# fpthink/PDGN

Hardware: AMD Instinct MI355X
Metric: generator+D step points/sec (B=35, 256->2048 pts) (higher is better)
Workload: dtype f32; 1 GPU; PDGNet_v2 G+D iteration (models/PDGNet_v2.py:171-256), chair-shaped synthetic batch, per-GPU batch 35, 256->2048 pts, random-init weights; global_batch=35, parallelism=dp1, losses_finite=True, hipgraph=False, issue=list

## Files before the change

### pdgn_amd/csrc/bnact.hip

```cpp
#include "common.h"

#include "bn_geom.h"
#define ACT_NONE 0
#define ACT_RELU 1
#define ACT_LEAKY 2

__device__ __forceinline__ float act_fwd(float z, int act) {
    if (act == ACT_RELU) return fmaxf(z, 0.f);
    if (act == ACT_LEAKY) return z > 0.f ? z : 0.01f * z;
    return z;
}
__device__ __forceinline__ float act_grad(float z, int act) {
    if (act == ACT_RELU) return z > 0.f ? 1.f : 0.f;
    if (act == ACT_LEAKY) return z > 0.f ? 1.f : 0.01f;
    return 1.f;
}

struct ClGeom {
    int cg, cgb, rl;
};

__global__ __launch_bounds__(BN_THREADS) void cl_stats_kernel(long long R, int C, int cgb, int rows_per_block,
                                                              const float *__restrict__ x,
                                                              float *__restrict__ part) {
// ... 635 lines not shown
    float acc[12];
#pragma unroll
    for (int i = 0; i < 12; ++i) acc[i] = 0.f;
    if (ok)
        for (long long m = m0 + rlane; m < m1; m += rl) {
            const size_t ox = (size_t)m * k * C + c, ou = (size_t)m * k * C + 2 * c;
            float2 xv[KM];
            float4 uv[KM / 2], wv[KM / 2], gv[KM / 2];
#pragma unroll
            for (int s = 0; s < KM; ++s)
                if (KT || s < k) xv[s] = *reinterpret_cast<const float2 *>(x + ox + (size_t)s * C);
#pragma unroll
            for (int p = 0; p < KM / 2; ++p)
                if (KT || p < P) {
                    uv[p] = *reinterpret_cast<const float4 *>(u + ou + (size_t)p * Cu);
                    if (w) wv[p] = *reinterpret_cast<const float4 *>(w + ou + (size_t)p * Cu);
                    gv[p] = *reinterpret_cast<const float4 *>(dy + ou + (size_t)p * Cu);
                }
            if (!w) {
                float h0[KM], h1[KM];
                float mx0 = -INFINITY, mx1 = -INFINITY;
#pragma unroll
                for (int s = 0; s < KM; ++s)
                    if (KT || s < k) {
                        h0[s] = act_fwd(__fmaf_rn(xv[s].x, scx.x, shx.x), act);
                        h1[s] = act_fwd(__fmaf_rn(xv[s].y, scx.y, shx.y), act);
                        mx0 = fmaxf(mx0, h0[s]);
                        mx1 = fmaxf(mx1, h1[s]);
                    }
                float e0 = 0.f, e1 = 0.f;
#pragma unroll
                for (int s = 0; s < KM; ++s)
                    if (KT || s < k) {
                        h0[s] = __expf(h0[s] - mx0);
                        h1[s] = __expf(h1[s] - mx1);
                        e0 += h0[s];
                        e1 += h1[s];
                    }
                const float i0 = 1.0f / e0, i1 = 1.0f / e1;
#pragma unroll
                for (int p = 0; p < KM / 2; ++p)
                    if (KT || p < P) wv[p] = make_float4(h0[p] * i0, h0[P + p] * i0, h1[p] * i1, h1[P + p] * i1);
            }
            float dot0 = 0.f, dot1 = 0.f;
#pragma unroll
            for (int p = 0; p < KM / 2; ++p)
                if (KT || p < P) {
                    const float u4[4] = {uv[p].x, uv[p].y, uv[p].z, uv[p].w}, w4[4] = {wv[p].x, wv[p].y, wv[p].z, wv[p].w};
                    const float g4[4] = {gv[p].x, gv[p].y, gv[p].z, gv[p].w};
                    const float s4[4] = {scu.x, scu.y, scu.z, scu.w}, h4[4] = {shu.x, shu.y, shu.z, shu.w};
                    const float m4[4] = {muu.x, muu.y, muu.z, muu.w}, i4[4] = {isu.x, isu.y, isu.z, isu.w};
                    const float a4[4] = {cau.x, cau.y, cau.z, cau.w}, b4[4] = {cbu.x, cbu.y, cbu.z, cbu.w};
                    float dW[4], o4[4];
#pragma unroll
                    for (int j = 0; j < 4; ++j) {
                        const float z = __fmaf_rn(u4[j], s4[j], h4[j]);
                        dW[j] = g4[j] * act_fwd(z, act);
                        const float dz = g4[j] * w4[j] * act_grad(z, act);
                        if (APPLY) o4[j] = __fmaf_rn(s4[j], dz, -a4[j]) - b4[j] * u4[j];
                        else { acc[4 + j] += dz; acc[8 + j] = __fmaf_rn(dz, (u4[j] - m4[j]) * i4[j], acc[8 + j]); }
                    }
                    if (APPLY) *reinterpret_cast<float4 *>(du + ou + (size_t)p * Cu) = make_float4(o4[0], o4[1], o4[2], o4[3]);
                    dot0 = __fmaf_rn(w4[0], dW[0], __fmaf_rn(w4[1], dW[1], dot0));
                    dot1 = __fmaf_rn(w4[2], dW[2], __fmaf_rn(w4[3], dW[3], dot1));
                    gv[p] = make_float4(dW[0], dW[1], dW[2], dW[3]);
                }
#pragma unroll
            for (int s = 0; s < KM; ++s)
                if (KT || s < k) {
                    const int p = s < P ? s : s - P;
                    const bool hi = s >= P;
                    const float w0 = hi ? wv[p].y : wv[p].x, g0 = hi ? gv[p].y : gv[p].x;
                    const float w1 = hi ? wv[p].w : wv[p].z, g1 = hi ? gv[p].w : gv[p].z;
                    const float da0 = w0 * (g0 - dot0), da1 = w1 * (g1 - dot1);
                    const float dz0 = da0 * act_grad(__fmaf_rn(xv[s].x, scx.x, shx.x), act);
                    const float dz1 = da1 * act_grad(__fmaf_rn(xv[s].y, scx.y, shx.y), act);
                    if (APPLY) {
                        float2 o;
                        o.x = __fmaf_rn(scx.x, dz0, -cax.x) - cbx.x * xv[s].x;
                        o.y = __fmaf_rn(scx.y, dz1, -cax.y) - cbx.y * xv[s].y;
                        *reinterpret_cast<float2 *>(dx + ox + (size_t)s * C) = o;
                    } else {
                        acc[0] += dz0; acc[1] += dz1;
                        acc[2] = __fmaf_rn(dz0, (xv[s].x - mux.x) * isx.x, acc[2]);
                        acc[3] = __fmaf_rn(dz1, (xv[s].y - mux.y) * isx.y, acc[3]);
                    }
                }
        }
    if (APPLY) return;
#pragma unroll
    for (int i = 0; i < 12; ++i) red[i][threadIdx.x] = acc[i];
    __syncthreads();
    if (rlane == 0 && ok) {
        for (int j = 1; j < rl; ++j)
#pragma unroll
            for (int i = 0; i < 12; ++i) acc[i] += red[i][j * cpb + cpl];
        float *px = part_x + (size_t)blockIdx.y * 2 * C, *pu = part_u + (size_t)blockIdx.y * 2 * Cu;
        *reinterpret_cast<float2 *>(px + c) = make_float2(acc[0], acc[1]);
        *reinterpret_cast<float2 *>(px + C + c) = make_float2(acc[2], acc[3]);
        *reinterpret_cast<float4 *>(pu + 2 * c) = make_float4(acc[4], acc[5], acc[6], acc[7]);
        *reinterpret_cast<float4 *>(pu + Cu + 2 * c) = make_float4(acc[8], acc[9], acc[10], acc[11]);
    }
}

static void bw_geometry(long long M, int C, int *cpb, int *gx, int *gy, int *mpb) {
    const int c2 = C / 2;
    int p = 1;
    while (p < c2 && p < BN_THREADS) p <<= 1;
    *cpb = p;
    *gx = (c2 + p - 1) / p;
    const int rl = BN_THREADS / p;
    long long want = 1024 / *gx;
    want = want < 1 ? 1 : want;
    long long rows = (M + want - 1) / want;
    rows = rows < (long long)rl * 4 ? (long long)rl * 4 : rows;
    rows = rows > 4096 ? 4096 : rows;
    rows = (rows + rl - 1) / rl * rl;
    *mpb = (int)rows;
    *gy = (int)((M + rows - 1) / rows);
}

extern "C" long long pdgn_bilateral_scratch_floats(long long m, int k, int c) {
    if (m < 1 || k < 2 || (k & 1) || k > BW_MAXK || c < 2 || (c & 1)) return PDGN_ERR_INVALID;
    int cpb, gx, gy, mpb;
    bw_geometry(m, c, &cpb, &gx, &gy, &mpb);
    return (long long)gy * 6 * c + 6 * c;
}

extern "C" int pdgn_bilateral_weighting_backward(long long m, int k, int c, int act, int training, const float *x,
                                                 const float *stats_x, const float *u, const float *stats_u,
                                                 const float *w, const float *dy, float *scratch, float *bsums_x,
                                                 float *bsums_u, float *dx, float *du, pdgn_stream_t stream) {
    if (m < 1 || k < 2 || (k & 1) || k > BW_MAXK || c < 4 || (c % 4) || act < 0 || act > 2) return PDGN_ERR_INVALID;
    hipStream_t s = (hipStream_t)stream;
    int cpb, gx, gy, mpb;
    bw_geometry(m, c, &cpb, &gx, &gy, &mpb);
    float *part_x = scratch, *part_u = part_x + (size_t)gy * 2 * c;
    float *coef_x = part_u + (size_t)gy * 4 * c, *coef_u = coef_x + 2 * c;
    const dim3 grid(gx, gy), block(BN_THREADS);
#define BW_LAUNCH(KT, AP)                                                                                              \
    hipLaunchKernelGGL((bilateral_bwd_kernel<KT, AP>), grid, block, 0, s, m, k, c, cpb, mpb, act, x, stats_x, u, stats_u, w, \
                       dy, part_x, part_u, coef_x, coef_u, dx, du)
    if (k == 10) BW_LAUNCH(10, false); else if (k == 4) BW_LAUNCH(4, false); else BW_LAUNCH(0, false);
    hipLaunchKernelGGL(cl_bwd_finalize_kernel, dim3(cdiv(c, FIN_CH)), dim3(FIN_CH * FIN_PL), 0, s, m * k, c, gy, training, part_x,
                       stats_x, bsums_x, coef_x);
    hipLaunchKernelGGL(cl_bwd_finalize_kernel, dim3(cdiv(2 * c, FIN_CH)), dim3(FIN_CH * FIN_PL), 0, s, m * (k / 2), 2 * c, gy,
                       training, part_u, stats_u, bsums_u, coef_u);
    if (k == 10) BW_LAUNCH(10, true); else if (k == 4) BW_LAUNCH(4, true); else BW_LAUNCH(0, true);
#undef BW_LAUNCH
    return pdgn_launch_status();
}

#define MP_SPLIT 16

__global__ __launch_bounds__(BN_THREADS) void cl_apply_max_kernel(int N, int C, int cgb, int act,
                                                                  const float *__restrict__ x,
                                                                  const float *__restrict__ stats,
                                                                  float *__restrict__ pmax, int32_t *__restrict__ parg) {
    __shared__ float smax[BN_THREADS][4];
    __shared__ int sarg[BN_THREADS][4];
    const int cgl = threadIdx.x % cgb, rlane = threadIdx.x / cgb, rl = BN_THREADS / cgb;
    const int cgi = blockIdx.x * cgb + cgl;
    const bool cok = cgi * 4 < C;
    const int b = blockIdx.z, sp = blockIdx.y;
    const int per = (N + MP_SPLIT - 1) / MP_SPLIT;
    const int n0 = sp * per, n1 = min(N, n0 + per);
    float best[4] = {-INFINITY, -INFINITY, -INFINITY, -INFINITY};
    int arg[4] = {n0, n0, n0, n0};
    if (cok) {
        float sc[4], sh[4];
        *reinterpret_cast<float4 *>(sc) = *reinterpret_cast<const float4 *>(stats + cgi * 4);
        *reinterpret_cast<float4 *>(sh) = *reinterpret_cast<const float4 *>(stats + C + cgi * 4);
        const float *X = x + ((size_t)b * N) * C + cgi * 4;
        for (int n = n0 + rlane; n < n1; n += rl) {
            float v[4];
            *reinterpret_cast<float4 *>(v) = *reinterpret_cast<const float4 *>(X + (size_t)n * C);
#pragma unroll
            for (int j = 0; j < 4; ++j) {
                const float y = act_fwd(__fmaf_rn(v[j], sc[j], sh[j]), act);
                if (y > best[j]) { best[j] = y; arg[j] = n; }
            }
        }
    }
#pragma unroll
    for (int j = 0; j < 4; ++j) { smax[threadIdx.x][j] = best[j]; sarg[threadIdx.x][j] = arg[j]; }
    __syncthreads();
    if (rlane == 0 && cok) {
        for (int q = 1; q < rl; ++q)
#pragma unroll
            for (int j = 0; j < 4; ++j) {
                const float y = smax[q * cgb + cgl][j];
                const int a = sarg[q * cgb + cgl][j];
                if (y > best[j] || (y == best[j] && a < arg[j])) { best[j] = y; arg[j] = a; }
            }
        const size_t o = ((size_t)b * MP_SPLIT + sp) * C + cgi * 4;
        *reinterpret_cast<float4 *>(pmax + o) = *reinterpret_cast<float4 *>(best);
        *reinterpret_cast<int4 *>(parg + o) = *reinterpret_cast<int4 *>(arg);
    }
}

__global__ void cl_max_finalize_kernel(int B, int C, const float *__restrict__ pmax, const int32_t *__restrict__ parg,
                                       float *__restrict__ ymax, int32_t *__restrict__ yarg) {
    const int e = blockIdx.x * blockDim.x + threadIdx.x;
    if (e >= B * C) return;
    const int b = e / C, c = e % C;
    float best = -INFINITY;
    int arg = 0;
    for (int s = 0; s < MP_SPLIT; ++s) {
        const float y = pmax[((size_t)b * MP_SPLIT + s) * C + c];
        if (y > best) { best = y; arg = parg[((size_t)b * MP_SPLIT + s) * C + c]; }
    }
    ymax[e] = best;
    yarg[e] = arg;
}

__global__ __launch_bounds__(BN_THREADS) void cl_stats_max_kernel(int N, int C, int cgb, const float *__restrict__ x,
                                                                  float *__restrict__ part, float *__restrict__ pmax,
                                                                  int32_t *__restrict__ pargmax, float *__restrict__ pmin,
                                                                  int32_t *__restrict__ pargmin) {
    __shared__ float4 red[4][BN_THREADS];
    __shared__ int4 redi[2][BN_THREADS];
    const int cgl = threadIdx.x % cgb, rlane = threadIdx.x / cgb, rl = BN_THREADS / cgb;
    const int cgi = blockIdx.x * cgb + cgl;
    const bool cok = cgi * 4 < C;
    const int b = blockIdx.z, sp = blockIdx.y;
    const int per = (N + MP_SPLIT - 1) / MP_SPLIT;
    const int n0 = sp * per, n1 = min(N, n0 + per);
    float s[4] = {0.f, 0.f, 0.f, 0.f}, q[4] = {0.f, 0.f, 0.f, 0.f};
    float mx[4] = {-INFINITY, -INFINITY, -INFINITY, -INFINITY}, mn[4] = {INFINITY, INFINITY, INFINITY, INFINITY};
    int amx[4] = {n0, n0, n0, n0}, amn[4] = {n0, n0, n0, n0};
    if (cok) {
        float pv[4];
        *reinterpret_cast<float4 *>(pv) = *reinterpret_cast<const float4 *>(x + cgi * 4);
        const float *X = x + ((size_t)b * N) * C + cgi * 4;
        for (int n = n0 + rlane; n < n1; n += rl) {
            float v[4];
            *reinterpret_cast<float4 *>(v) = *reinterpret_cast<const float4 *>(X + (size_t)n * C);
#pragma unroll
            for (int j = 0; j < 4; ++j) {
                const float d = v[j] - pv[j];
                s[j] += d;
                q[j] = __fmaf_rn(d, d, q[j]);
                if (v[j] > mx[j]) { mx[j] = v[j]; amx[j] = n; }
                if (v[j] < mn[j]) { mn[j] = v[j]; amn[j] = n; }
            }
        }
    }
    red[0][threadIdx.x] = make_float4(s[0], s[1], s[2], s[3]);
    red[1][threadIdx.x] = make_float4(q[0], q[1], q[2], q[3]);
    red[2][threadIdx.x] = make_float4(mx[0], mx[1], mx[2], mx[3]);
    red[3][threadIdx.x] = make_float4(mn[0], mn[1], mn[2], mn[3]);
    redi[0][threadIdx.x] = make_int4(amx[0], amx[1], amx[2], amx[3]);
    redi[1][threadIdx.x] = make_int4(amn[0], amn[1], amn[2], amn[3]);
    __syncthreads();
    if (rlane || !cok) return;
    for (int k = 1; k < rl; ++k) {
        const int t = k * cgb + cgl;
        const float *a = &red[0][t].x, *bq = &red[1][t].x, *c2 = &red[2][t].x, *d2 = &red[3][t].x;
        const int *i2 = &redi[0][t].x, *j2 = &redi[1][t].x;
#pragma unroll
        for (int j = 0; j < 4; ++j) {
            s[j] += a[j];
            q[j] += bq[j];
            if (c2[j] > mx[j] || (c2[j] == mx[j] && i2[j] < amx[j])) { mx[j] = c2[j]; amx[j] = i2[j]; }
            if (d2[j] < mn[j] || (d2[j] == mn[j] && j2[j] < amn[j])) { mn[j] = d2[j]; amn[j] = j2[j]; }
        }
    }
    const size_t blk = (size_t)b * MP_SPLIT + sp;
    float *P = part + blk * 2 * C;
    *reinterpret_cast<float4 *>(P + cgi * 4) = make_float4(s[0], s[1], s[2], s[3]);
    *reinterpret_cast<float4 *>(P + C + cgi * 4) = make_float4(q[0], q[1], q[2], q[3]);
    const size_t o = blk * C + cgi * 4;
    *reinterpret_cast<float4 *>(pmax + o) = make_float4(mx[0], mx[1], mx[2], mx[3]);
    *reinterpret_cast<int4 *>(pargmax + o) = make_int4(amx[0], amx[1], amx[2], amx[3]);
    *reinterpret_cast<float4 *>(pmin + o) = make_float4(mn[0], mn[1], mn[2], mn[3]);
    *reinterpret_cast<int4 *>(pargmin + o) = make_int4(amn[0], amn[1], amn[2], amn[3]);
}

__global__ void cl_max_pick_kernel(int B, int C, int act, const float *__restrict__ stats, const float *__restrict__ pmax,
                                   const int32_t *__restrict__ pargmax, const float *__restrict__ pmin,
                                   const int32_t *__restrict__ pargmin, float *__restrict__ ymax, int32_t *__restrict__ yarg) {
    const int e = blockIdx.x * blockDim.x + threadIdx.x;
    if (e >= B * C) return;
    const int b = e / C, c = e - b * C;
    const float sc = stats[c], sh = stats[C + c];
    const bool up = sc >= 0.f;
    const float *pv = up ? pmax : pmin;
    const int32_t *pa = up ? pargmax : pargmin;
    float best = pv[((size_t)b * MP_SPLIT) * C + c];
    int arg = pa[((size_t)b * MP_SPLIT) * C + c];
    for (int s = 1; s < MP_SPLIT; ++s) {
        const float v = pv[((size_t)b * MP_SPLIT + s) * C + c];
        if (up ? v > best : v < best) { best = v; arg = pa[((size_t)b * MP_SPLIT + s) * C + c]; }
    }
    ymax[e] = act_fwd(__fmaf_rn(best, sc, sh), act);
    yarg[e] = arg;
}

__global__ __launch_bounds__(256) void cl_max_bwd_sums_kernel(int B, int N, int C, int act, int training,
                                                              const float *__restrict__ x, const float *__restrict__ dout,
                                                              const int32_t *__restrict__ yarg, const float *__restrict__ stats,
                                                              float *__restrict__ dz, float *__restrict__ bsums,
                                                              float *__restrict__ coef, float *__restrict__ zero, int nzero) {
    __shared__ double p1[16][17], p2[16][17];
    for (int e = blockIdx.x * 256 + threadIdx.x; e < nzero; e += gridDim.x * 256) zero[e] = 0.f;
    const int cl = threadIdx.x & 15, bl = threadIdx.x >> 4;
    const int c = blockIdx.x * 16 + cl;
    double s1 = 0, s2 = 0;
    float sc = 0.f, mu = 0.f, is = 0.f;
    if (c < C) {
        sc = stats[c];
        mu = stats[2 * C + c];
        is = stats[3 * C + c];
        const float sh = stats[C + c];
        for (int b = bl; b < B; b += 16) {
            const int n = yarg[b * C + c];
            const float v = x[((size_t)b * N + n) * C + c];
            const float g = dout[b * C + c] * act_grad(__fmaf_rn(v, sc, sh), act);
            dz[b * C + c] = g;
            s1 += g;
            s2 += (double)g * (double)((v - mu) * is);
        }
    }
    p1[bl][cl] = s1;
    p2[bl][cl] = s2;
    __syncthreads();
    if (bl || c >= C) return;
    for (int q = 1; q < 16; ++q) { s1 += p1[q][cl]; s2 += p2[q][cl]; }
    bsums[c] = (float)s1;
    bsums[C + c] = (float)s2;
    float ca = 0.f, cb = 0.f;
    if (training) {
        const double R = (double)B * (double)N;
        cb = sc * is * (float)(s2 / R);
        ca = sc * (float)(s1 / R) - cb * mu;
    }
    coef[c] = ca;
    coef[C + c] = cb;
}

__global__ __launch_bounds__(BN_THREADS) void cl_max_bwd_apply_kernel(int N, int C, int cgb, const float *__restrict__ x,
                                                                      const float *__restrict__ stats,
                                                                      const float *__restrict__ coef,
                                                                      const float *__restrict__ dz,
                                                                      const int32_t *__restrict__ yarg,
                                                                      float *__restrict__ dx) {
    const int cgl = threadIdx.x % cgb, rlane = threadIdx.x / cgb, rl = BN_THREADS / cgb;
    const int cgi = blockIdx.x * cgb + cgl;
    if (cgi * 4 >= C) return;
    const int b = blockIdx.z, sp = blockIdx.y;
    const int per = (N + MP_SPLIT - 1) / MP_SPLIT;
    const int n0 = sp * per, n1 = min(N, n0 + per);
    float sc[4], ca[4], cb[4], g[4];
    int arg[4];
    *reinterpret_cast<float4 *>(sc) = *reinterpret_cast<const float4 *>(stats + cgi * 4);
    *reinterpret_cast<float4 *>(ca) = *reinterpret_cast<const float4 *>(coef + cgi * 4);
    *reinterpret_cast<float4 *>(cb) = *reinterpret_cast<const float4 *>(coef + C + cgi * 4);
    *reinterpret_cast<float4 *>(g) = *reinterpret_cast<const float4 *>(dz + (size_t)b * C + cgi * 4);
    *reinterpret_cast<int4 *>(arg) = *reinterpret_cast<const int4 *>(yarg + (size_t)b * C + cgi * 4);
    const size_t base = ((size_t)b * N) * C + cgi * 4;
    for (int n = n0 + rlane; n < n1; n += rl) {
        float v[4], o[4];
        *reinterpret_cast<float4 *>(v) = *reinterpret_cast<const float4 *>(x + base + (size_t)n * C);
#pragma unroll
        for (int j = 0; j < 4; ++j) o[j] = (n == arg[j] ? sc[j] * g[j] : 0.f) - ca[j] - cb[j] * v[j];
        *reinterpret_cast<float4 *>(dx + base + (size_t)n * C) = *reinterpret_cast<float4 *>(o);
    }
}

static void mp_geometry(int C, int *cgb, int *gx) {
    const int cg = C / 4;
    int p = 1;
    while (p < cg && p < 64) p <<= 1;
    *cgb = p;
    *gx = (cg + p - 1) / p;
}

extern "C" long long pdgn_bn_maxpool_scratch_floats(int b, int c) { return 2LL * b * MP_SPLIT * c; }

extern "C" int pdgn_bn_act_maxpool(int b, int n, int c, int act, const float *x, const float *stats, float *scratch,
                                   float *ymax, int32_t *yarg, pdgn_stream_t stream) {
    if (b < 1 || n < 1 || c < 4 || c % 4 || act < 0 || act > 2 || b > 65535) return PDGN_ERR_INVALID;
    hipStream_t s = (hipStream_t)stream;
    int cgb, gx;
    mp_geometry(c, &cgb, &gx);
    float *pmax = scratch;
    int32_t *parg = reinterpret_cast<int32_t *>(scratch + (size_t)b * MP_SPLIT * c);
    hipLaunchKernelGGL(cl_apply_max_kernel, dim3(gx, MP_SPLIT, b), dim3(BN_THREADS), 0, s, n, c, cgb, act, x, stats, pmax, parg);
    hipLaunchKernelGGL(cl_max_finalize_kernel, dim3(cdiv((long long)b * c, 256)), dim3(256), 0, s, b, c, pmax, parg, ymax, yarg);
    return pdgn_launch_status();
}

extern "C" long long pdgn_bn_stats_maxpool_scratch_floats(int b, int c) { return 6LL * b * MP_SPLIT * c; }

extern "C" int pdgn_bn_stats_act_maxpool(int b, int n, int c, int act, float eps, float momentum, const float *x, const float *gamma,
                                         const float *beta, const float *pre_bias, float *running_mean, float *running_var,
                                         float *scratch, float *stats, float *ymax, int32_t *yarg, pdgn_stream_t stream) {
    if (b < 1 || n < 1 || c < 4 || c % 4 || act < 0 || act > 2 || b > 65535) return PDGN_ERR_INVALID;
    hipStream_t s = (hipStream_t)stream;
    int cgb, gx;
    mp_geometry(c, &cgb, &gx);
    const size_t bc = (size_t)b * MP_SPLIT * c;
    float *part = scratch, *pmax = part + 2 * bc, *pmin = pmax + 2 * bc;
    int32_t *pargmax = reinterpret_cast<int32_t *>(pmax + bc), *pargmin = reinterpret_cast<int32_t *>(pmin + bc);
    hipLaunchKernelGGL(cl_stats_max_kernel, dim3(gx, MP_SPLIT, b), dim3(BN_THREADS), 0, s, n, c, cgb, x, part, pmax, pargmax, pmin,
                       pargmin);
    hipLaunchKernelGGL(cl_finalize_kernel, dim3(cdiv(c, FIN_CH)), dim3(FIN_CH * FIN_PL), 0, s, (long long)b * n, c, b * MP_SPLIT, eps,
                       momentum, part, gamma, beta, pre_bias, running_mean, running_var, stats, x);
    hipLaunchKernelGGL(cl_max_pick_kernel, dim3(cdiv((long long)b * c, 256)), dim3(256), 0, s, b, c, act, stats, pmax, pargmax, pmin,
                       pargmin, ymax, yarg);
    return pdgn_launch_status();
}

extern "C" int pdgn_bn_act_maxpool_backward(int b, int n, int c, int act, int training, const float *x,
                                            const float *dout, const int32_t *yarg, const float *stats, float *scratch,
                                            float *bsums, float *dx, pdgn_stream_t stream) {
    if (b < 1 || n < 1 || c < 4 || c % 4 || act < 0 || act > 2 || b > 65535) return PDGN_ERR_INVALID;
    hipStream_t s = (hipStream_t)stream;
    float *dz = scratch, *coef = scratch + (size_t)b * c;
    hipLaunchKernelGGL(cl_max_bwd_sums_kernel, dim3(cdiv(c, 16)), dim3(256), 0, s, b, n, c, act, training, x, dout, yarg,
                       stats, dz, bsums, coef, nullptr, 0);
    int cgb, gx;
    mp_geometry(c, &cgb, &gx);
    hipLaunchKernelGGL(cl_max_bwd_apply_kernel, dim3(gx, MP_SPLIT, b), dim3(BN_THREADS), 0, s, n, c, cgb, x, stats, coef, dz,
                       yarg, dx);
    return pdgn_launch_status();
}

#define CF_TILE 32
#define CF_CSPLIT 8
#define CF_RSPLIT 32

__global__ __launch_bounds__(256) void cf_gram_kernel(int C, int K, const float *__restrict__ W, int ldw,
                                                      const float *__restrict__ coef, float *__restrict__ Gneg,
                                                      float *__restrict__ vneg) {
    __shared__ float part[3][64][20];
    const int t = threadIdx.x, o = t & 63, sl = __builtin_amdgcn_readfirstlane(t >> 6);
    const int i = blockIdx.y * CF_TILE + (o >> 3) * 4, j = blockIdx.x * CF_TILE + (o & 7) * 4;
    const bool ok = i < K && j < K, do_v = blockIdx.y == 0 && (o >> 3) == 0 && j < K;
    const int ii = min(i, K - 4), jj = min(j, K - 4);
    const int nsl = CF_CSPLIT * 4, per = (C + nsl - 1) / nsl;
    const int c0 = (blockIdx.z * 4 + sl) * per, c1 = min(C, c0 + per);
    const float *cb = coef + C;
    float acc[4][4] = {}, av[4] = {};
    for (int c = c0; c < c1; c += 8) {
        float4 wi[8], wj[8];
#pragma unroll
        for (int u = 0; u < 8; ++u) {
            const float *w = W + (size_t)min(c + u, c1 - 1) * ldw;
            wi[u] = *reinterpret_cast<const float4 *>(w + ii);
            wj[u] = *reinterpret_cast<const float4 *>(w + jj);
        }
        __builtin_amdgcn_sched_barrier(0);
#pragma unroll
        for (int u = 0; u < 8; ++u) {
            const int cc = min(c + u, c1 - 1);
            const float live = c + u < c1 ? 1.f : 0.f;
            const float s = cb[cc] * live, a = coef[cc] * live;
            const float x[4] = {wi[u].x * s, wi[u].y * s, wi[u].z * s, wi[u].w * s};
            const float y[4] = {wj[u].x, wj[u].y, wj[u].z, wj[u].w};
#pragma unroll
            for (int p = 0; p < 4; ++p)
#pragma unroll
                for (int q = 0; q < 4; ++q) acc[p][q] = __fmaf_rn(x[p], y[q], acc[p][q]);
#pragma unroll
            for (int q = 0; q < 4; ++q) av[q] = __fmaf_rn(a, y[q], av[q]);
        }
    }
    if (sl) {
#pragma unroll
        for (int p = 0; p < 4; ++p)
#pragma unroll
            for (int q = 0; q < 4; ++q) part[sl - 1][o][p * 4 + q] = acc[p][q];
#pragma unroll
        for (int q = 0; q < 4; ++q) part[sl - 1][o][16 + q] = av[q];
    }
    __syncthreads();
    if (sl) return;
#pragma unroll
    for (int w = 0; w < 3; ++w) {
#pragma unroll
        for (int p = 0; p < 4; ++p)
#pragma unroll
            for (int q = 0; q < 4; ++q) acc[p][q] += part[w][o][p * 4 + q];
#pragma unroll
        for (int q = 0; q < 4; ++q) av[q] += part[w][o][16 + q];
    }
    if (ok)
#pragma unroll
        for (int p = 0; p < 4; ++p)
#pragma unroll
            for (int q = 0; q < 4; ++q) atomicAdd(&Gneg[(size_t)(i + p) * K + j + q], -acc[p][q]);
    if (do_v)
#pragma unroll
        for (int q = 0; q < 4; ++q) atomicAdd(&vneg[j + q], -av[q]);
}

__global__ __launch_bounds__(256) void cf_scatter_kernel(int N, int C, int K, const float *__restrict__ W, int ldw,
                                                         const float *__restrict__ stats, const float *__restrict__ dz,
                                                         const int32_t *__restrict__ yarg, float *__restrict__ dh) {
    extern __shared__ unsigned char cf_lds[];
    __shared__ unsigned int ndist;
    const int maxd = min(N, C);
    unsigned short *table = reinterpret_cast<unsigned short *>(cf_lds);
    unsigned short *rows = table + N;
    unsigned short *args = rows + maxd;
    unsigned int *cnt = reinterpret_cast<unsigned int *>(cf_lds + (((size_t)(N + maxd + C) * 2 + 15) & ~(size_t)15));
    float *cf = reinterpret_cast<float *>(cnt + 256);
    const int t = threadIdx.x, b = blockIdx.y;
    const int32_t *arg = yarg + (size_t)b * C;
    for (int n = t; n < N; n += 256) table[n] = 0;
    __syncthreads();
    for (int c = t; c < C; c += 256) {
        const int a = arg[c];
        table[a] = 1;
        args[c] = (unsigned short)a;
        cf[c] = stats[c] * dz[(size_t)b * C + c];
    }
    __syncthreads();
    const int per = (N + 255) / 256, lo = t * per, hi = min(N, lo + per);
    unsigned int mine = 0;
    for (int n = lo; n < hi; ++n) mine += table[n];
    cnt[t] = mine;
    __syncthreads();
    if (t < 64) {
        const unsigned int v0 = cnt[4 * t], v1 = cnt[4 * t + 1], v2 = cnt[4 * t + 2], v3 = cnt[4 * t + 3];
        const unsigned int s = v0 + v1 + v2 + v3;
        unsigned int incl = s;
#pragma unroll
        for (int d = 1; d < 64; d <<= 1) {
            const unsigned int up = __shfl_up(incl, d, 64);
            if (t >= d) incl += up;
        }
        const unsigned int ex = incl - s;
        cnt[4 * t] = ex;
        cnt[4 * t + 1] = ex + v0;
        cnt[4 * t + 2] = ex + v0 + v1;
        cnt[4 * t + 3] = ex + v0 + v1 + v2;
    }
    __syncthreads();
    unsigned int at = cnt[t];
    for (int n = lo; n < hi; ++n)
        if (table[n]) rows[at++] = (unsigned short)n;
    if (t == 255) ndist = at;
    __syncthreads();
    const int nd = (int)ndist, lane = t & 63, wv = t >> 6;
    const bool lok = lane * 4 < K;
    const int col = min(lane * 4, K - 4);
    for (int r = blockIdx.x * 4 + wv; r < nd; r += CF_RSPLIT * 4) {
        const int n = rows[r];
        float *dst = dh + ((size_t)b * N + n) * K + col;
        const float4 cur = *reinterpret_cast<const float4 *>(dst);
        float4 acc = make_float4(0.f, 0.f, 0.f, 0.f);
        for (int c0 = 0; c0 < C; c0 += 64) {
            unsigned long long m = __ballot(c0 + lane < C && args[min(c0 + lane, C - 1)] == n);
            while (m) {
                const int c = c0 + __builtin_ctzll(m);
                m &= m - 1;
                const float g = cf[c];
                const float4 w = *reinterpret_cast<const float4 *>(W + (size_t)c * ldw + col);
                acc.x = __fmaf_rn(g, w.x, acc.x);
                acc.y = __fmaf_rn(g, w.y, acc.y);
                acc.z = __fmaf_rn(g, w.z, acc.z);
                acc.w = __fmaf_rn(g, w.w, acc.w);
            }
        }
        if (lok) *reinterpret_cast<float4 *>(dst) = make_float4(cur.x + acc.x, cur.y + acc.y, cur.z + acc.z, cur.w + acc.w);
    }
}

static size_t cf_scatter_lds(int n, int c) {
    const int maxd = n < c ? n : c;
    return (((size_t)(n + maxd + c) * 2 + 15) & ~(size_t)15) + 256 * 4 + (size_t)c * 4;
}

#define CFS_THREADS 1024
__global__ __launch_bounds__(CFS_THREADS) void cf_colsum_kernel(long long rows, int K, const float *__restrict__ h, int ldh,
                                                                float *__restrict__ hs) {
    __shared__ float4 red[CFS_THREADS];
    const int kg = K / 4, cg = threadIdx.x % kg, rl = threadIdx.x / kg, nrl = CFS_THREADS / kg;
    const long long per = (rows + gridDim.x - 1) / gridDim.x, r0 = blockIdx.x * per, r1 = min(rows, r0 + per);
    float4 acc = make_float4(0.f, 0.f, 0.f, 0.f);
    for (long long r = r0 + rl; r < r1; r += 8 * nrl) {
        float4 v[8];
#pragma unroll
        for (int u = 0; u < 8; ++u) {
            const long long rr = r + (long long)u * nrl;
            v[u] = rr < r1 ? *reinterpret_cast<const float4 *>(h + rr * ldh + cg * 4) : make_float4(0.f, 0.f, 0.f, 0.f);
        }
#pragma unroll
        for (int u = 0; u < 8; ++u) { acc.x += v[u].x; acc.y += v[u].y; acc.z += v[u].z; acc.w += v[u].w; }
    }
    red[threadIdx.x] = acc;
    __syncthreads();
    if (rl) return;
    for (int q = 1; q < nrl; ++q) {
        const float4 v = red[q * kg + cg];
        acc.x += v.x; acc.y += v.y; acc.z += v.z; acc.w += v.w;
    }
    atomicAdd(&hs[cg * 4], acc.x); atomicAdd(&hs[cg * 4 + 1], acc.y); atomicAdd(&hs[cg * 4 + 2], acc.z); atomicAdd(&hs[cg * 4 + 3], acc.w);
}

__global__ __launch_bounds__(256) void cf_dw_kernel(int B, int N, int C, int K, const float *__restrict__ h, int ldh,
                                                    const int32_t *__restrict__ yarg, const float *__restrict__ stats,
                                                    const float *__restrict__ dz, const float *__restrict__ coef,
                                                    const float *__restrict__ hs, const float *__restrict__ T,
                                                    float *__restrict__ dW, int lddw) {
    const int lane = threadIdx.x & 63, c = blockIdx.x * 4 + (threadIdx.x >> 6);
    if (c >= C || lane * 4 >= K) return;
    const int col = lane * 4;
    const float sc = stats[c];
    float4 acc = make_float4(0.f, 0.f, 0.f, 0.f);
    for (int b0 = 0; b0 < B; b0 += 8) {
        float4 v[8];
        float g[8];
#pragma unroll
        for (int u = 0; u < 8; ++u) {
            const int b = min(b0 + u, B - 1);
            g[u] = b0 + u < B ? sc * dz[(size_t)b * C + c] : 0.f;
            v[u] = *reinterpret_cast<const float4 *>(h + ((size_t)b * N + yarg[(size_t)b * C + c]) * ldh + col);
        }
#pragma unroll
        for (int u = 0; u < 8; ++u) {
            acc.x = __fmaf_rn(g[u], v[u].x, acc.x);
            acc.y = __fmaf_rn(g[u], v[u].y, acc.y);
            acc.z = __fmaf_rn(g[u], v[u].z, acc.z);
            acc.w = __fmaf_rn(g[u], v[u].w, acc.w);
        }
    }
    const float ca = coef[c], cb = coef[C + c];
    const float4 s = *reinterpret_cast<const float4 *>(hs + col), t = *reinterpret_cast<const float4 *>(T + (size_t)c * K + col);
    *reinterpret_cast<float4 *>(dW + (size_t)c * lddw + col) =
        make_float4(acc.x - ca * s.x - cb * t.x, acc.y - ca * s.y - cb * t.y, acc.z - ca * s.z - cb * t.z, acc.w - ca * s.w - cb * t.w);
}

extern "C" long long pdgn_dense_bn_maxpool_backward_scratch(int b, int c, int k) {
    return (long long)b * c + 2LL * c + 2LL * ((long long)k * k + k) + (long long)c * k;
}

extern "C" int pdgn_dense_bn_maxpool_backward(int b, int n, int c, int k, int act, const float *x, const float *dout,
                                              const int32_t *yarg, const float *stats, const float *h, int ldh, const float *W,
                                              int ldw, float *scratch, float *dh, float *dW, int lddw, float *bsums,
                                              pdgn_stream_t stream) {
    if (b < 1 || n < 1 || n > 65535 || c < 4 || c % 4 || k < 4 || k % 4 || k > 256 || ldw % 4 || ((uintptr_t)W & 15) ||
        ((uintptr_t)dh & 15) || act < 0 || act > 2 || b > 65535 || cf_scatter_lds(n, c) > 64 * 1024)
        return PDGN_ERR_INVALID;
    if (dW && (k < 16 || (k & (k - 1)) || ldh % 4 || lddw % 4 || ((uintptr_t)h & 15) || ((uintptr_t)dW & 15)))
        return PDGN_ERR_INVALID;
    hipStream_t s = (hipStream_t)stream;
    const size_t kk = (size_t)k * k;
    float *dz = scratch, *coef = dz + (size_t)b * c, *G = coef + 2 * (size_t)c, *v = G + kk, *H = v + k, *hs = H + kk, *T = hs + k;
    float *bs = bsums ? bsums : T;
    hipLaunchKernelGGL(cl_max_bwd_sums_kernel, dim3(cdiv(c, 16)), dim3(256), 0, s, b, n, c, act, 1, x, dout, yarg, stats, dz, bs,
                       coef, G, (int)(2 * (kk + k)));
    int rc = pdgn_launch_status();
    if (rc) return rc;
    if (dh) {
        const int gt = cdiv(k, CF_TILE);
        hipLaunchKernelGGL(cf_gram_kernel, dim3(gt, gt, CF_CSPLIT), dim3(256), 0, s, c, k, W, ldw, coef, G, v);
        if ((rc = pdgn_launch_status())) return rc;
        if ((rc = pdgn_gemm_nt((long long)b * n, k, k, h, ldh, G, k, v, nullptr, 0, dh, k, nullptr, stream))) return rc;
        hipLaunchKernelGGL(cf_scatter_kernel, dim3(CF_RSPLIT, b), dim3(256), cf_scatter_lds(n, c), s, n, c, k, W, ldw, stats, dz,
                           yarg, dh);
        if ((rc = pdgn_launch_status())) return rc;
    }
    if (dW) {
        const long long rows = (long long)b * n;
        hipLaunchKernelGGL(cf_colsum_kernel, dim3(rows >= 32768 ? 128 : (rows >= 8192 ? 64 : 16)), dim3(CFS_THREADS), 0, s, rows, k, h, ldh, hs);
        if ((rc = pdgn_launch_status())) return rc;
        if ((rc = pdgn_gemm_tn_big(rows, k, k, h, ldh, h, ldh, H, 1, stream))) return rc;
        if ((rc = pdgn_gemm_nt(c, k, k, W, ldw, H, k, nullptr, nullptr, 0, T, k, nullptr, stream))) return rc;
        hipLaunchKernelGGL(cf_dw_kernel, dim3(cdiv(c, 4)), dim3(256), 0, s, b, n, c, k, h, ldh, yarg, stats, dz, coef, hs, T, dW, lddw);
        rc = pdgn_launch_status();
    }
    return rc;
}

extern "C" long long pdgn_dense_bn_maxpool_input_grad_scratch(int b, int c, int k) {
    return pdgn_dense_bn_maxpool_backward_scratch(b, c, k);
}

extern "C" int pdgn_dense_bn_maxpool_input_grad(int b, int n, int c, int k, int act, const float *x, const float *dout,
                                                const int32_t *yarg, const float *stats, const float *h, int ldh,
                                                const float *W, int ldw, float *scratch, float *dh, pdgn_stream_t stream) {
    return pdgn_dense_bn_maxpool_backward(b, n, c, k, act, x, dout, yarg, stats, h, ldh, W, ldw, scratch, dh, nullptr, 4, nullptr,
                                          stream);
}

__global__ __launch_bounds__(256) void group_colsum_kernel(long long group_rows, int C, const float *__restrict__ x, long long ldx,
                                                           float *__restrict__ out) {
    __shared__ float4 red[256];
    const int kg = C / 4, per_pass = kg < 256 ? kg : 256;
    const int cgl = threadIdx.x % per_pass, rl = threadIdx.x / per_pass, nrl = 256 / per_pass;
    const long long g = blockIdx.y;
    const long long per = (group_rows + gridDim.x - 1) / gridDim.x, r0 = blockIdx.x * per, r1 = min(group_rows, r0 + per);
    const float *X = x + g * group_rows * ldx;
    for (int c0 = 0; c0 < kg; c0 += per_pass) {
        const int cg = c0 + cgl;
        float4 acc = make_float4(0.f, 0.f, 0.f, 0.f);
        for (long long r = r0 + rl; r < r1; r += 8 * nrl) {
            float4 v[8];
#pragma unroll
            for (int u = 0; u < 8; ++u) {
                const long long rr = r + (long long)u * nrl;
                v[u] = rr < r1 ? *reinterpret_cast<const float4 *>(X + rr * ldx + cg * 4) : make_float4(0.f, 0.f, 0.f, 0.f);
            }
#pragma unroll
            for (int u = 0; u < 8; ++u) { acc.x += v[u].x; acc.y += v[u].y; acc.z += v[u].z; acc.w += v[u].w; }
        }
        __syncthreads();
        red[threadIdx.x] = acc;
        __syncthreads();
        if (rl == 0) {
            for (int q = 1; q < nrl; ++q) {
                const float4 v = red[q * per_pass + cgl];
                acc.x += v.x; acc.y += v.y; acc.z += v.z; acc.w += v.w;
            }
            float *o = out + g * C + cg * 4;
            if (gridDim.x == 1) *reinterpret_cast<float4 *>(o) = acc;
            else { atomicAdd(o, acc.x); atomicAdd(o + 1, acc.y); atomicAdd(o + 2, acc.z); atomicAdd(o + 3, acc.w); }
        }
    }
}

extern "C" int pdgn_group_colsum(long long groups, long long group_rows, int c, const float *x, long long ldx, float *out,
                                 pdgn_stream_t stream) {
    if (groups < 1 || group_rows < 1 || c < 16 || c > 1024 || (c & (c - 1)) || ldx < c || ldx % 4 || ((uintptr_t)x & 15) ||
        ((uintptr_t)out & 15) || groups > 65535)
        return PDGN_ERR_INVALID;
    const int kg = c / 4, nrl = kg < 256 ? 256 / kg : 1;
    long long splits = 1024 / groups;
    splits = splits > 128 ? 128 : splits;
    const long long max_splits = group_rows / (8LL * nrl * 8) > 0 ? group_rows / (8LL * nrl * 8) : 1;
    splits = splits < 1 ? 1 : (splits > max_splits ? max_splits : splits);
    hipLaunchKernelGGL(group_colsum_kernel, dim3((unsigned)splits, (unsigned)groups), dim3(256), 0, (hipStream_t)stream, group_rows, c, x,
                       ldx, out);
    return pdgn_launch_status();
}
```

Baseline: 3.115 million points/s.

## Rework maxpool-backward scatter, colsum partials, dW gather and unroll maxpool reductions

```diff
diff --git a/pdgn_amd/csrc/bnact.hip b/pdgn_amd/csrc/bnact.hip
--- a/pdgn_amd/csrc/bnact.hip
+++ b/pdgn_amd/csrc/bnact.hip
@@ -811,6 +811,7 @@
 }
 
 #define MP_SPLIT 16
+#define MP_UNROLL 8
 
 __global__ __launch_bounds__(BN_THREADS) void cl_apply_max_kernel(int N, int C, int cgb, int act,
                                                                   const float *__restrict__ x,
@@ -831,15 +832,24 @@
         *reinterpret_cast<float4 *>(sc) = *reinterpret_cast<const float4 *>(stats + cgi * 4);
         *reinterpret_cast<float4 *>(sh) = *reinterpret_cast<const float4 *>(stats + C + cgi * 4);
         const float *X = x + ((size_t)b * N) * C + cgi * 4;
-        for (int n = n0 + rlane; n < n1; n += rl) {
-            float v[4];
-            *reinterpret_cast<float4 *>(v) = *reinterpret_cast<const float4 *>(X + (size_t)n * C);
+        auto take = [&](const float4 &r, int n) {
+            const float v[4] = {r.x, r.y, r.z, r.w};
 #pragma unroll
             for (int j = 0; j < 4; ++j) {
                 const float y = act_fwd(__fmaf_rn(v[j], sc[j], sh[j]), act);
                 if (y > best[j]) { best[j] = y; arg[j] = n; }
             }
-        }
+        };
+        int n = n0 + rlane;
+        for (; n + (MP_UNROLL - 1) * rl < n1; n += MP_UNROLL * rl) {
+            float4 v[MP_UNROLL];
+#pragma unroll
+            for (int u = 0; u < MP_UNROLL; ++u) v[u] = *reinterpret_cast<const float4 *>(X + (size_t)(n + u * rl) * C);
+            __builtin_amdgcn_sched_barrier(0);
+#pragma unroll
+            for (int u = 0; u < MP_UNROLL; ++u) take(v[u], n + u * rl);
+        }
+        for (; n < n1; n += rl) take(*reinterpret_cast<const float4 *>(X + (size_t)n * C), n);
     }
 #pragma unroll
     for (int j = 0; j < 4; ++j) { smax[threadIdx.x][j] = best[j]; sarg[threadIdx.x][j] = arg[j]; }
@@ -892,9 +902,8 @@
         float pv[4];
         *reinterpret_cast<float4 *>(pv) = *reinterpret_cast<const float4 *>(x + cgi * 4);
         const float *X = x + ((size_t)b * N) * C + cgi * 4;
-        for (int n = n0 + rlane; n < n1; n += rl) {
-            float v[4];
-            *reinterpret_cast<float4 *>(v) = *reinterpret_cast<const float4 *>(X + (size_t)n * C);
+        auto take = [&](const float4 &r, int n) {
+            const float v[4] = {r.x, r.y, r.z, r.w};
 #pragma unroll
             for (int j = 0; j < 4; ++j) {
                 const float d = v[j] - pv[j];
@@ -903,7 +912,17 @@
                 if (v[j] > mx[j]) { mx[j] = v[j]; amx[j] = n; }
                 if (v[j] < mn[j]) { mn[j] = v[j]; amn[j] = n; }
             }
-        }
+        };
+        int n = n0 + rlane;
+        for (; n + (MP_UNROLL - 1) * rl < n1; n += MP_UNROLL * rl) {
+            float4 v[MP_UNROLL];
+#pragma unroll
+            for (int u = 0; u < MP_UNROLL; ++u) v[u] = *reinterpret_cast<const float4 *>(X + (size_t)(n + u * rl) * C);
+            __builtin_amdgcn_sched_barrier(0);
+#pragma unroll
+            for (int u = 0; u < MP_UNROLL; ++u) take(v[u], n + u * rl);
+        }
+        for (; n < n1; n += rl) take(*reinterpret_cast<const float4 *>(X + (size_t)n * C), n);
     }
     red[0][threadIdx.x] = make_float4(s[0], s[1], s[2], s[3]);
     red[1][threadIdx.x] = make_float4(q[0], q[1], q[2], q[3]);
@@ -936,21 +955,34 @@
     *reinterpret_cast<int4 *>(pargmin + o) = make_int4(amn[0], amn[1], amn[2], amn[3]);
 }
 
-__global__ void cl_max_pick_kernel(int B, int C, int act, const float *__restrict__ stats, const float *__restrict__ pmax,
-                                   const int32_t *__restrict__ pargmax, const float *__restrict__ pmin,
-                                   const int32_t *__restrict__ pargmin, float *__restrict__ ymax, int32_t *__restrict__ yarg) {
+__global__ __launch_bounds__(256) void cl_max_pick_kernel(int B, int C, int act, const float *__restrict__ stats,
+                                                          const float *__restrict__ pmax, const int32_t *__restrict__ pargmax,
+                                                          const float *__restrict__ pmin, const int32_t *__restrict__ pargmin,
+                                                          float *__restrict__ ymax, int32_t *__restrict__ yarg) {
     const int e = blockIdx.x * blockDim.x + threadIdx.x;
     if (e >= B * C) return;
     const int b = e / C, c = e - b * C;
+    const size_t o = ((size_t)b * MP_SPLIT) * C + c;
+    float vx[MP_SPLIT], vn[MP_SPLIT];
+    int ax[MP_SPLIT], an[MP_SPLIT];
+#pragma unroll
+    for (int s = 0; s < MP_SPLIT; ++s) {
+        vx[s] = pmax[o + (size_t)s * C];
+        ax[s] = pargmax[o + (size_t)s * C];
+        vn[s] = pmin[o + (size_t)s * C];
+        an[s] = pargmin[o + (size_t)s * C];
+    }
     const float sc = stats[c], sh = stats[C + c];
+    __builtin_amdgcn_sched_barrier(0);
     const bool up = sc >= 0.f;
-    const float *pv = up ? pmax : pmin;
-    const int32_t *pa = up ? pargmax : pargmin;
-    float best = pv[((size_t)b * MP_SPLIT) * C + c];
-    int arg = pa[((size_t)b * MP_SPLIT) * C + c];
+    float best = up ? vx[0] : vn[0];
+    int arg = up ? ax[0] : an[0];
+#pragma unroll
     for (int s = 1; s < MP_SPLIT; ++s) {
-        const float v = pv[((size_t)b * MP_SPLIT + s) * C + c];
-        if (up ? v > best : v < best) { best = v; arg = pa[((size_t)b * MP_SPLIT + s) * C + c]; }
+        const float v = up ? vx[s] : vn[s];
+        const bool take = up ? v > best : v < best;
+        best = take ? v : best;
+        arg = take ? (up ? ax[s] : an[s]) : arg;
     }
     ymax[e] = act_fwd(__fmaf_rn(best, sc, sh), act);
     yarg[e] = arg;
@@ -1088,7 +1120,7 @@
 
 #define CF_TILE 32
 #define CF_CSPLIT 8
-#define CF_RSPLIT 32
+#define CF_RSPLIT 8
 
 __global__ __launch_bounds__(256) void cf_gram_kernel(int C, int K, const float *__restrict__ W, int ldw,
                                                       const float *__restrict__ coef, float *__restrict__ Gneg,
@@ -1155,32 +1187,38 @@
         for (int q = 0; q < 4; ++q) atomicAdd(&vneg[j + q], -av[q]);
 }
 
-__global__ __launch_bounds__(256) void cf_scatter_kernel(int N, int C, int K, const float *__restrict__ W, int ldw,
-                                                         const float *__restrict__ stats, const float *__restrict__ dz,
-                                                         const int32_t *__restrict__ yarg, float *__restrict__ dh) {
+#define CFSC_THREADS 1024
+__global__ __launch_bounds__(CFSC_THREADS) void cf_scatter_kernel(int N, int C, int K, const float *__restrict__ W, int ldw,
+                                                                  const float *__restrict__ stats, const float *__restrict__ dz,
+                                                                  const int32_t *__restrict__ yarg, float *__restrict__ dh) {
     extern __shared__ unsigned char cf_lds[];
     __shared__ unsigned int ndist;
     const int maxd = min(N, C);
     unsigned short *table = reinterpret_cast<unsigned short *>(cf_lds);
+    unsigned int *tw = reinterpret_cast<unsigned int *>(cf_lds);
     unsigned short *rows = table + N;
-    unsigned short *args = rows + maxd;
+    unsigned short *list = rows + maxd;
     unsigned int *cnt = reinterpret_cast<unsigned int *>(cf_lds + (((size_t)(N + maxd + C) * 2 + 15) & ~(size_t)15));
     float *cf = reinterpret_cast<float *>(cnt + 256);
     const int t = threadIdx.x, b = blockIdx.y;
     const int32_t *arg = yarg + (size_t)b * C;
-    for (int n = t; n < N; n += 256) table[n] = 0;
-    __syncthreads();
-    for (int c = t; c < C; c += 256) {
+    for (int n = t; n < (N + 1) / 2; n += CFSC_THREADS) tw[n] = 0;
+    __syncthreads();
+    for (int c = t; c < C; c += CFSC_THREADS) {
         const int a = arg[c];
-        table[a] = 1;
-        args[c] = (unsigned short)a;
+        atomicAdd(&tw[a >> 1], 1u << ((a & 1) * 16));
         cf[c] = stats[c] * dz[(size_t)b * C + c];
     }
     __syncthreads();
-    const int per = (N + 255) / 256, lo = t * per, hi = min(N, lo + per);
-    unsigned int mine = 0;
-    for (int n = lo; n < hi; ++n) mine += table[n];
-    cnt[t] = mine;
+    const int per = (N + 255) / 256, lo = min(N, t * per), hi = t < 256 ? min(N, lo + per) : lo;
+    if (t < 256) {
+        unsigned int mine = 0;
+        for (int n = lo; n < hi; ++n) {
+            const unsigned int k = table[n];
+            mine += k ? 0x10000u + k : 0u;
+        }
+        cnt[t] = mine;
+    }
     __syncthreads();
     if (t < 64) {
         const unsigned int v0 = cnt[4 * t], v1 = cnt[4 * t + 1], v2 = cnt[4 * t + 2], v3 = cnt[4 * t + 3];
@@ -1198,30 +1236,69 @@
         cnt[4 * t + 3] = ex + v0 + v1 + v2;
     }
     __syncthreads();
-    unsigned int at = cnt[t];
-    for (int n = lo; n < hi; ++n)
-        if (table[n]) rows[at++] = (unsigned short)n;
-    if (t == 255) ndist = at;
-    __syncthreads();
-    const int nd = (int)ndist, lane = t & 63, wv = t >> 6;
+    if (t < 256) {
+        unsigned int at = cnt[t] >> 16, off = cnt[t] & 0xffffu;
+        for (int n = lo; n < hi; ++n) {
+            const unsigned int k = table[n];
+            if (k) {
+                rows[at++] = (unsigned short)n;
+                table[n] = (unsigned short)off;
+                off += k;
+            }
+        }
+        if (t == 255) ndist = at;
+    }
+    __syncthreads();
+    for (int c = t; c < C; c += CFSC_THREADS) {
+        const int a = arg[c], sh = (a & 1) * 16;
+        const unsigned int old = atomicAdd(&tw[a >> 1], 1u << sh);
+        list[(old >> sh) & 0xffffu] = (unsigned short)c;
+    }
+    __syncthreads();
+    const int nd = (int)ndist, lane = t & 63, wv = __builtin_amdgcn_readfirstlane(t >> 6);
     const bool lok = lane * 4 < K;
     const int col = min(lane * 4, K - 4);
-    for (int r = blockIdx.x * 4 + wv; r < nd; r += CF_RSPLIT * 4) {
+    const float *Wc = W + col;
+    for (int r = blockIdx.x * (CFSC_THREADS / 64) + wv; r < nd; r += gridDim.x * (CFSC_THREADS / 64)) {
         const int n = rows[r];
+        const int e1 = table[n], e0 = r ? table[rows[r - 1]] : 0, L = __builtin_amdgcn_readfirstlane(e1 - e0);
         float *dst = dh + ((size_t)b * N + n) * K + col;
         const float4 cur = *reinterpret_cast<const float4 *>(dst);
         float4 acc = make_float4(0.f, 0.f, 0.f, 0.f);
-        for (int c0 = 0; c0 < C; c0 += 64) {
-            unsigned long long m = __ballot(c0 + lane < C && args[min(c0 + lane, C - 1)] == n);
-            while (m) {
-                const int c = c0 + __builtin_ctzll(m);
-                m &= m - 1;
-                const float g = cf[c];
-                const float4 w = *reinterpret_cast<const float4 *>(W + (size_t)c * ldw + col);
-                acc.x = __fmaf_rn(g, w.x, acc.x);
-                acc.y = __fmaf_rn(g, w.y, acc.y);
-                acc.z = __fmaf_rn(g, w.z, acc.z);
-                acc.w = __fmaf_rn(g, w.w, acc.w);
+        auto add_rows = [&](int ch, float g, int m) {
+            for (int j = 0; j < m; j += 8) {
+                float4 w[8];
+#pragma unroll
+                for (int u = 0; u < 8; ++u) {
+                    const int c = __builtin_amdgcn_readlane(ch, min(j + u, m - 1));
+                    w[u] = *reinterpret_cast<const float4 *>(Wc + (size_t)c * ldw);
+                }
+                __builtin_amdgcn_sched_barrier(0);
+#pragma unroll
+                for (int u = 0; u < 8; ++u)
+                    if (j + u < m) {
+                        const float gu = __int_as_float(__builtin_amdgcn_readlane(__float_as_int(g), j + u));
+                        acc.x = __fmaf_rn(gu, w[u].x, acc.x);
+                        acc.y = __fmaf_rn(gu, w[u].y, acc.y);
+                        acc.z = __fmaf_rn(gu, w[u].z, acc.z);
+                        acc.w = __fmaf_rn(gu, w[u].w, acc.w);
+                    }
+            }
+        };
+        if (L <= 64) {
+            const int mine = lane < L ? (int)list[e0 + lane] : 0x7fffffff;
+            int rank = 0;
+            for (int j = 0; j < L; ++j) rank += __builtin_amdgcn_readlane(mine, j) < mine ? 1 : 0;
+            const int ch = __builtin_amdgcn_ds_permute((lane < L ? rank : lane) * 4, mine);
+            add_rows(ch, lane < L ? cf[ch] : 0.f, L);
+        } else {
+            for (int c0 = 0; c0 < C; c0 += 64) {
+                const bool hit = c0 + lane < C && arg[min(c0 + lane, C - 1)] == n;
+                const unsigned long long m = __ballot(hit);
+                const int k = __popcll(m), before = __popcll(m & ((1ull << lane) - 1ull));
+                if (!k) continue;
+                const int ch = __builtin_amdgcn_ds_permute((hit ? before : k + lane - before) * 4, c0 + lane);
+                add_rows(ch, lane < k ? cf[ch] : 0.f, k);
             }
         }
         if (lok) *reinterpret_cast<float4 *>(dst) = make_float4(cur.x + acc.x, cur.y + acc.y, cur.z + acc.z, cur.w + acc.w);
@@ -1234,8 +1311,9 @@
 }
 
 #define CFS_THREADS 1024
+#define CFS_PART 64
 __global__ __launch_bounds__(CFS_THREADS) void cf_colsum_kernel(long long rows, int K, const float *__restrict__ h, int ldh,
-                                                                float *__restrict__ hs) {
+                                                                float *__restrict__ hs, int nparts) {
     __shared__ float4 red[CFS_THREADS];
     const int kg = K / 4, cg = threadIdx.x % kg, rl = threadIdx.x / kg, nrl = CFS_THREADS / kg;
     const long long per = (rows + gridDim.x - 1) / gridDim.x, r0 = blockIdx.x * per, r1 = min(rows, r0 + per);
@@ -1257,44 +1335,72 @@
         const float4 v = red[q * kg + cg];
         acc.x += v.x; acc.y += v.y; acc.z += v.z; acc.w += v.w;
     }
-    atomicAdd(&hs[cg * 4], acc.x); atomicAdd(&hs[cg * 4 + 1], acc.y); atomicAdd(&hs[cg * 4 + 2], acc.z); atomicAdd(&hs[cg * 4 + 3], acc.w);
-}
+    float *o = hs + (size_t)(blockIdx.x % nparts) * K + cg * 4;
+    atomicAdd(o, acc.x); atomicAdd(o + 1, acc.y); atomicAdd(o + 2, acc.z); atomicAdd(o + 3, acc.w);
+}
+
+static int cf_colsum_grid(long long rows) { return rows >= 32768 ? 8 * CFS_PART : (rows >= 8192 ? 64 : 16); }
 
 __global__ __launch_bounds__(256) void cf_dw_kernel(int B, int N, int C, int K, const float *__restrict__ h, int ldh,
                                                     const int32_t *__restrict__ yarg, const float *__restrict__ stats,
                                                     const float *__restrict__ dz, const float *__restrict__ coef,
-                                                    const float *__restrict__ hs, const float *__restrict__ T,
+                                                    const float *__restrict__ hs, int nparts, const float *__restrict__ T,
                                                     float *__restrict__ dW, int lddw) {
-    const int lane = threadIdx.x & 63, c = blockIdx.x * 4 + (threadIdx.x >> 6);
-    if (c >= C || lane * 4 >= K) return;
-    const int col = lane * 4;
-    const float sc = stats[c];
+    __shared__ float4 hsum[64];
+    const int lane = threadIdx.x & 63, wv = __builtin_amdgcn_readfirstlane(threadIdx.x >> 6);
+    const int c = min(blockIdx.x * 4 + wv, C - 1);
+    const bool live = blockIdx.x * 4 + wv < C && lane * 4 < K;
+    const int col = min(lane * 4, K - 4);
+    if (wv == 0) {
+        float4 s = make_float4(0.f, 0.f, 0.f, 0.f);
+        for (int p = 0; p < nparts; p += 16) {
+            float4 v[16];
+#pragma unroll
+            for (int u = 0; u < 16; ++u) v[u] = *reinterpret_cast<const float4 *>(hs + (size_t)min(p + u, nparts - 1) * K + col);
+            __builtin_amdgcn_sched_barrier(0);
+#pragma unroll
+            for (int u = 0; u < 16; ++u)
+                if (p + u < nparts) { s.x += v[u].x; s.y += v[u].y; s.z += v[u].z; s.w += v[u].w; }
+        }
+        hsum[lane] = s;
+    }
+    const float sc = stats[c], ca = coef[c], cb = coef[C + c];
+    const float4 t = *reinterpret_cast<const float4 *>(T + (size_t)c * K + col);
+    const float *hc = h + col;
     float4 acc = make_float4(0.f, 0.f, 0.f, 0.f);
-    for (int b0 = 0; b0 < B; b0 += 8) {
-        float4 v[8];
-        float g[8];
-#pragma unroll
-        for (int u = 0; u < 8; ++u) {
-            const int b = min(b0 + u, B - 1);
-            g[u] = b0 + u < B ? sc * dz[(size_t)b * C + c] : 0.f;
-            v[u] = *reinterpret_cast<const float4 *>(h + ((size_t)b * N + yarg[(size_t)b * C + c]) * ldh + col);
-        }
-#pragma unroll
-        for (int u = 0; u < 8; ++u) {
-            acc.x = __fmaf_rn(g[u], v[u].x, acc.x);
-            acc.y = __fmaf_rn(g[u], v[u].y, acc.y);
-            acc.z = __fmaf_rn(g[u], v[u].z, acc.z);
-            acc.w = __fmaf_rn(g[u], v[u].w, acc.w);
-        }
-    }
-    const float ca = coef[c], cb = coef[C + c];
-    const float4 s = *reinterpret_cast<const float4 *>(hs + col), t = *reinterpret_cast<const float4 *>(T + (size_t)c * K + col);
-    *reinterpret_cast<float4 *>(dW + (size_t)c * lddw + col) =
-        make_float4(acc.x - ca * s.x - cb * t.x, acc.y - ca * s.y - cb * t.y, acc.z - ca * s.z - cb * t.z, acc.w - ca * s.w - cb * t.w);
+    for (int b0 = 0; b0 < B; b0 += 64) {
+        const int m = min(64, B - b0), bl = min(b0 + lane, B - 1);
+        const int al = yarg[(size_t)bl * C + c];
+        const float gl = sc * dz[(size_t)bl * C + c];
+        for (int j = 0; j < m; j += 8) {
+            float4 v[8];
+#pragma unroll
+            for (int u = 0; u < 8; ++u) {
+                const int jj = min(j + u, m - 1);
+                const int a = __builtin_amdgcn_readlane(al, jj);
+                v[u] = *reinterpret_cast<const float4 *>(hc + ((size_t)(b0 + jj) * N + a) * ldh);
+            }
+            __builtin_amdgcn_sched_barrier(0);
+#pragma unroll
+            for (int u = 0; u < 8; ++u)
+                if (j + u < m) {
+                    const float g = __int_as_float(__builtin_amdgcn_readlane(__float_as_int(gl), j + u));
+                    acc.x = __fmaf_rn(g, v[u].x, acc.x);
+                    acc.y = __fmaf_rn(g, v[u].y, acc.y);
+                    acc.z = __fmaf_rn(g, v[u].z, acc.z);
+                    acc.w = __fmaf_rn(g, v[u].w, acc.w);
+                }
+        }
+    }
+    __syncthreads();
+    const float4 s = hsum[lane];
+    if (live)
+        *reinterpret_cast<float4 *>(dW + (size_t)c * lddw + col) =
+            make_float4(acc.x - ca * s.x - cb * t.x, acc.y - ca * s.y - cb * t.y, acc.z - ca * s.z - cb * t.z, acc.w - ca * s.w - cb * t.w);
 }
 
 extern "C" long long pdgn_dense_bn_maxpool_backward_scratch(int b, int c, int k) {
-    return (long long)b * c + 2LL * c + 2LL * ((long long)k * k + k) + (long long)c * k;
+    return (long long)b * c + 2LL * c + 2LL * (long long)k * k + k + (long long)CFS_PART * k + (long long)c * k;
 }
 
 extern "C" int pdgn_dense_bn_maxpool_backward(int b, int n, int c, int k, int act, const float *x, const float *dout,
@@ -1308,10 +1414,11 @@
         return PDGN_ERR_INVALID;
     hipStream_t s = (hipStream_t)stream;
     const size_t kk = (size_t)k * k;
-    float *dz = scratch, *coef = dz + (size_t)b * c, *G = coef + 2 * (size_t)c, *v = G + kk, *H = v + k, *hs = H + kk, *T = hs + k;
+    float *dz = scratch, *coef = dz + (size_t)b * c, *G = coef + 2 * (size_t)c, *v = G + kk, *H = v + k, *hs = H + kk;
+    float *T = hs + (size_t)CFS_PART * k;
     float *bs = bsums ? bsums : T;
     hipLaunchKernelGGL(cl_max_bwd_sums_kernel, dim3(cdiv(c, 16)), dim3(256), 0, s, b, n, c, act, 1, x, dout, yarg, stats, dz, bs,
-                       coef, G, (int)(2 * (kk + k)));
+                       coef, G, (int)(2 * kk + k + (size_t)CFS_PART * k));
     int rc = pdgn_launch_status();
     if (rc) return rc;
     if (dh) {
@@ -1319,17 +1426,19 @@
         hipLaunchKernelGGL(cf_gram_kernel, dim3(gt, gt, CF_CSPLIT), dim3(256), 0, s, c, k, W, ldw, coef, G, v);
         if ((rc = pdgn_launch_status())) return rc;
         if ((rc = pdgn_gemm_nt((long long)b * n, k, k, h, ldh, G, k, v, nullptr, 0, dh, k, nullptr, stream))) return rc;
-        hipLaunchKernelGGL(cf_scatter_kernel, dim3(CF_RSPLIT, b), dim3(256), cf_scatter_lds(n, c), s, n, c, k, W, ldw, stats, dz,
-                           yarg, dh);
+        hipLaunchKernelGGL(cf_scatter_kernel, dim3(CF_RSPLIT, b), dim3(CFSC_THREADS), cf_scatter_lds(n, c), s, n, c, k, W, ldw, stats,
+                           dz, yarg, dh);
         if ((rc = pdgn_launch_status())) return rc;
     }
     if (dW) {
         const long long rows = (long long)b * n;
-        hipLaunchKernelGGL(cf_colsum_kernel, dim3(rows >= 32768 ? 128 : (rows >= 8192 ? 64 : 16)), dim3(CFS_THREADS), 0, s, rows, k, h, ldh, hs);
+        const int gs = cf_colsum_grid(rows);
+        hipLaunchKernelGGL(cf_colsum_kernel, dim3(gs), dim3(CFS_THREADS), 0, s, rows, k, h, ldh, hs, gs / 8);
         if ((rc = pdgn_launch_status())) return rc;
         if ((rc = pdgn_gemm_tn_big(rows, k, k, h, ldh, h, ldh, H, 1, stream))) return rc;
         if ((rc = pdgn_gemm_nt(c, k, k, W, ldw, H, k, nullptr, nullptr, 0, T, k, nullptr, stream))) return rc;
-        hipLaunchKernelGGL(cf_dw_kernel, dim3(cdiv(c, 4)), dim3(256), 0, s, b, n, c, k, h, ldh, yarg, stats, dz, coef, hs, T, dW, lddw);
+        hipLaunchKernelGGL(cf_dw_kernel, dim3(cdiv(c, 4)), dim3(256), 0, s, b, n, c, k, h, ldh, yarg, stats, dz, coef, hs,
+                           gs / 8, T, dW, lddw);
         rc = pdgn_launch_status();
     }
     return rc;
```

Result: no change. 3.115 million points/s (median of 2 runs) (+0.0%).
